# efirdc/Segmentation-Pipeline

Measured on AMD Instinct MI355X. Metric: 3D patches/sec (128³, 4ch) train+infer at 1/2/4/8 MI355X; Dice vs CPU ref, higher is better.
Workload: dtype f32 (tensors, results and accumulation; the products of the 3x3x3 convolutions with >= 8 input channels run as six bf16 MFMAs on an EXACT three-way bf16 split of both f32 operands -- error vs f64 equal to the f32 MFMA kernels', profiles/r04_f32x3_accuracy.txt; the same step on v_mfma_f32_32x32x2_f32

## Files before the change

### include/m355seg.h

```cpp
#ifndef M355SEG_H
#define M355SEG_H

#include <stddef.h>
#include <stdint.h>

#ifdef __cplusplus
extern "C" {
#endif

#define M355_ABI_VERSION 3

enum {
  M355_OK = 0,
  M355_EINVALID_ARG = -1,
  M355_EUNSUPPORTED = -2,
  M355_ELAUNCH = -3,
  M355_EWORKSPACE = -4
};

enum { M355_F32 = 0 };

enum { M355_COMPUTE_F32 = 0, M355_COMPUTE_BF16 = 1, M355_COMPUTE_F16 = 2, M355_COMPUTE_F32X3 = 3 };

enum { M355_ACT_NONE = 0, M355_ACT_RELU = 1, M355_ACT_LEAKY_RELU = 2, M355_ACT_ELU = 3, M355_ACT_GELU = 4,
// ... 65 lines not shown
                               size_t workspace_bytes, void* stream);

int m355_conv3d_plan(const m355_conv3d_desc* d, int32_t which, int32_t* out4);

int m355_conv3d_launch_plan(int32_t entry, const m355_conv3d_desc* d, const int64_t* batch_strides, const uint64_t* pointers,
                            size_t workspace_bytes, int64_t* out12);

size_t m355_conv3d_bwd_data_workspace(const m355_conv3d_desc* d);
int m355_conv3d_bwd_data(const m355_conv3d_desc* d, const float* dy, const float* w,
                         float* dx, void* workspace, size_t workspace_bytes, void* stream);

size_t m355_conv3d_bwd_weight_workspace(const m355_conv3d_desc* d);
int m355_conv3d_bwd_weight(const m355_conv3d_desc* d, const float* x, const float* dy,
                           float* dw, float* dbias,
                           void* workspace, size_t workspace_bytes, void* stream);

size_t m355_conv_transpose3d_workspace(const m355_conv3d_desc* d);
int m355_conv_transpose3d_fwd(const m355_conv3d_desc* d, const float* x, const float* w,
                              const float* bias, float* y,
                              void* workspace, size_t workspace_bytes, void* stream);
int m355_conv_transpose3d_bwd_data(const m355_conv3d_desc* d, const float* dy, const float* w,
                                   float* dx, void* workspace, size_t workspace_bytes,
                                   void* stream);
int m355_conv_transpose3d_bwd_weight(const m355_conv3d_desc* d, const float* x, const float* dy,
                                     float* dw, float* dbias,
                                     void* workspace, size_t workspace_bytes, void* stream);

int m355_conv_transpose3d_plan(const m355_conv3d_desc* d, int32_t which, const void* y_side, int32_t* out4);

int32_t m355_conv_transpose3d_x3_bwd_supported(const m355_conv3d_desc* d, const void* y_side);
// ... 521 lines not shown
```

### segmentation-pipeline_amd/_lib.py

```python
import ctypes as C
import os

_HERE = os.path.dirname(os.path.abspath(__file__))
LIB_PATH = os.environ.get("M355_LIB_PATH") or os.path.join(_HERE, "libm355seg.so")

M355_OK = 0
M355_EUNSUPPORTED = -2
ACT_NONE, ACT_RELU, ACT_LEAKY_RELU = 0, 1, 2
ACT_ELU, ACT_GELU, ACT_GELU_TANH, ACT_SILU = 3, 4, 5, 6
COMPUTE_F32, COMPUTE_BF16, COMPUTE_F16, COMPUTE_F32X3 = 0, 1, 2, 3
CONV_W_PACKED, CONV_SOFTMAX, CONV_SIGMOID = 1, 2, 4


class ConvDesc(C.Structure):
    _fields_ = [
        ("N", C.c_int32), ("Cin", C.c_int32), ("Cout", C.c_int32),
        ("D", C.c_int32), ("H", C.c_int32), ("W", C.c_int32),
        ("k", C.c_int32), ("stride", C.c_int32), ("pad", C.c_int32), ("out_pad", C.c_int32),
        ("x_batch_stride", C.c_int64), ("y_batch_stride", C.c_int64),
        ("compute", C.c_int32), ("flags", C.c_int32),
    ]


class PackItem(C.Structure):
# ... 163 lines not shown
    "m355_upsample_trilinear2x_fwd_h16": (C.c_int, [_P, _P, _i32, _i32, _i32, _i32, _i32, _i64, _i64, _i32, _P]),
    "m355_upsample_trilinear2x_bwd_h16": (C.c_int, [_P, _P, _i32, _i32, _i32, _i32, _i32, _i64, _i64, _i32, _P]),
    "m355_act16_channel_scale": (C.c_int, [_P, _P, _P, _i32, _i32, _i64, _i64, _i64, _i32, _P]),
    "m355_space_to_depth2_h16": (C.c_int, [_P, _P, _i32, _i32, _i32, _i32, _i32, _i64, _i64, _i32, _P]),
    "m355_depth_to_space2_h16": (C.c_int, [_P, _P, _i32, _i32, _i32, _i32, _i32, _i64, _i64, _i32, _P]),
    "m355_conv_transpose3d_h16_bwd_supported": (_i32, [_CD]),
    "m355_conv_transpose3d_h16_bwd_workspace": (_sz, [_CD]),
    "m355_conv_transpose3d_bwd_data_h16": (C.c_int, [_CD, _P, _i64, _P, _P, _i64, _i32, _P]),
    "m355_conv_transpose3d_bwd_weight_h16": (C.c_int, [_CD, _P, _i64, _P, _i64, _P, _P, _f32, _i32, _P, _sz, _P]),
    "m355_conv3d_plan": (C.c_int, [_CD, _i32, C.POINTER(C.c_int32)]),
    "m355_conv3d_launch_plan": (C.c_int, [_i32, _CD, C.POINTER(_i64), C.POINTER(C.c_uint64), _sz, C.POINTER(_i64)]),
    "m355_conv3d_bwd_data_workspace": (_sz, [_CD]),
    "m355_conv3d_bwd_data": (C.c_int, [_CD, _P, _P, _P, _P, _sz, _P]),
    "m355_conv3d_bwd_weight_workspace": (_sz, [_CD]),
    "m355_conv3d_bwd_weight": (C.c_int, [_CD, _P, _P, _P, _P, _P, _sz, _P]),
    "m355_conv_transpose3d_workspace": (_sz, [_CD]),
    "m355_conv_transpose3d_plan": (C.c_int, [_CD, _i32, _P, C.POINTER(C.c_int32)]),
    "m355_conv_transpose3d_fwd": (C.c_int, [_CD, _P, _P, _P, _P, _P, _sz, _P]),
    "m355_conv_transpose3d_bwd_data": (C.c_int, [_CD, _P, _P, _P, _P, _sz, _P]),
    "m355_conv_transpose3d_bwd_weight": (C.c_int, [_CD, _P, _P, _P, _P, _P, _sz, _P]),
    "m355_conv_transpose3d_fwd_h16": (C.c_int, [_CD, _P, _i64, _P, _P, _P, _i64, _i32, _P]),
    "m355_conv_transpose3d_x3_bwd_supported": (_i32, [_CD, _P]),
    "m355_conv_transpose3d_x3_bwd_workspace": (_sz, [_CD]),
    "m355_conv_transpose3d_x3_bwd_plan": (C.c_int, [_CD, _i32, _P, C.POINTER(C.c_int32)]),
    "m355_conv_transpose3d_bwd_data_x3": (C.c_int, [_CD, _P, _P, _P, _P, _sz, _P]),
    "m355_conv_transpose3d_bwd_weight_x3": (C.c_int, [_CD, _P, _P, _P, _P, _P, _sz, _P]),
    "m355_norm_num_stats": (_i64, [_ND]),
    "m355_norm_workspace": (_sz, [_ND]),
    "m355_norm_plan": (C.c_int, [_ND, _i32, C.POINTER(C.c_int32)]),
    "m355_norm_stats": (C.c_int, [_ND, _P, _P, _P, _P, _P, _f32, _P, _sz, _P]),
# ... 226 lines not shown
```

### segmentation-pipeline_amd/csrc/abi.cpp

```cpp
#include "common.hpp"
#include <map>
#include <mutex>
#include <tuple>
#include <utility>

namespace m355 {
static thread_local char g_err[512] = "";
void set_error(const char* fmt, ...) {
  va_list ap;
  va_start(ap, fmt);
  vsnprintf(g_err, sizeof(g_err), fmt, ap);
  va_end(ap);
}

static int env_int(const char* name, int dflt) {
  const char* v = getenv(name);
  if (!v || !*v) return dflt;
  return atoi(v);
}
static Tuning read_tuning() {
  Tuning t;
  t.conv_ntw = env_int("M355_CONV_NTW", 0);
  t.conv_ksplit = env_int("M355_CONV_KSPLIT", 0);
  t.conv_slots = env_int("M355_CONV_SLOTS", 0);
  t.conv_persistent = env_int("M355_CONV_PERSISTENT", 1);
  t.no_small = env_int("M355_NO_SMALL", 0);
  t.smallcout_valu = env_int("M355_SMALLCOUT_VALU", 1);
  t.f32x3 = env_int("M355_F32X3", 1);
  t.f32x3_bww = env_int("M355_F32X3_BWW", 1);
  t.f32x3_edge = env_int("M355_F32X3_EDGE", 0);
  t.f32x3_convt = env_int("M355_F32X3_CONVT", 1);
  t.f32x3_convt_bwd = env_int("M355_F32X3_CONVT_BWD", 1);
  t.bww_nsplit = env_int("M355_BWW_NSPLIT", 0);
  t.bww_gen = env_int("M355_BWW_GEN", 2);
  t.bww_queue = env_int("M355_BWW_QUEUE", 1);
  t.h16_persistent = env_int("M355_H16_PERSISTENT", 1);
  t.tile16 = env_int("M355_TILE16", 1);
  t.convt_h16 = env_int("M355_CONVT_H16", 1);
  t.h16_w8 = env_int("M355_H16_W8", 1);
  t.h16_oneshot = env_int("M355_H16_ONESHOT", 1);
  t.h16_xcd = env_int("M355_H16_XCD", 1);
  t.conv_cube = env_int("M355_CONV_CUBE", 3);
  t.h16_order = env_int("M355_H16_ORDER", 3);
  t.fuse_softmax = env_int("M355_FUSE_SOFTMAX", 1);
  t.convt_wgs = env_int("M355_CONVT_WGS", 0);
  t.h16_stagger = env_int("M355_H16_STAGGER", 2);
  return t;
// ... 104 lines not shown
```

### segmentation-pipeline_amd/csrc/common.hpp

```cpp
#pragma once
#include <hip/hip_runtime.h>
#include <stdint.h>
#include <stdio.h>
#include <stdarg.h>
#include <stdlib.h>
#include <algorithm>
#include "../../include/m355seg.h"

namespace m355 {

void set_error(const char* fmt, ...);

static inline int64_t ceil_div(int64_t a, int64_t b) { return (a + b - 1) / b; }
static inline int64_t round_up(int64_t a, int64_t b) { return ceil_div(a, b) * b; }

static inline int check_launch(const char* what) {
  hipError_t e = hipGetLastError();
  if (e != hipSuccess) {
    set_error("%s: launch failed: %s", what, hipGetErrorString(e));
    return M355_ELAUNCH;
  }
  return M355_OK;
}

// ... 31 lines not shown
  }
  return r;
}

__device__ __forceinline__ float sigmoid_f32(float v) { return 1.f / (1.f + expf(-v)); }

struct Tuning {
  int conv_ntw = 0, conv_ksplit = 0, conv_slots = 0, conv_persistent = 1;
  int no_small = 0, smallcout_valu = 1, bww_nsplit = 0, bww_gen = 2, bww_queue = 1, h16_persistent = 1, tile16 = 1, convt_h16 = 1, h16_w8 = 1, h16_oneshot = 1, h16_xcd = 1;
  int conv_cube = 3, h16_order = 3;
  int fuse_softmax = 1;
  int f32x3 = 1;
  int f32x3_bww = 1;
  int f32x3_edge = 0;
  int f32x3_convt = 1;
  int f32x3_convt_bwd = 1;
  int convt_wgs = 0;
  int h16_stagger = 2;
};
const Tuning& tuning();

static inline int64_t dense_or(int64_t stride, int64_t dense) { return stride ? stride : dense; }

int num_cus();

int* queue_state(hipStream_t st);
int* overflow_flag();

}
```

### segmentation-pipeline_amd/csrc/conv3d.hip

```cpp
#include "conv3d_common.hpp"

namespace m355 {

__global__ void pack_w3_kernel(const float* __restrict__ w, float* __restrict__ wp, int Cout,
                               int Cin, int kin_pad, int mout_pad, int transpose, int* __restrict__ counter) {
  if (counter && blockIdx.x == 0 && threadIdx.x < 16) counter[threadIdx.x] = 0;
  pack_w3_body(w, wp, Cout, Cin, kin_pad, mout_pad, transpose, blockIdx.x, gridDim.x);
}

template <int NTW, int GX>
__global__ __launch_bounds__(256, 1) void conv3_mfma_fwd_kernel(
    const float* __restrict__ x, const float* __restrict__ wp, const float* __restrict__ bias,
    const float* __restrict__ add, float* __restrict__ y, float* __restrict__ slab, int Cin,
    int Cout, int D, int H, int W, int cout_pad, int ty_tiles, int tx_tiles, int nchunks,
    int ksplit, int64_t xbs, int64_t ybs, int64_t slab_stride, float* __restrict__ stat, int otiles, int order) {
  using T = FwdTile<NTW, GX>;
  constexpr int GY = T::GY, TZ = T::TZ, TY = T::TY, TX = T::TX, RS = T::RS, PS = T::PS,
                CS = T::CS, CC = T::CC;
  constexpr int XE = CC * CS;
  constexpr int XPER = (XE + 255) / 256;
  constexpr int WE4 = CC * 27 * 8;
  constexpr int WPER = (WE4 + 255) / 256;
  __shared__ float xs[2][XE];
  __shared__ __attribute__((aligned(16))) float ws[2][CC * 27 * 32];
// ... 1500 lines not shown
    } else {
      for (int64_t s = begin + threadIdx.x; s < end; s += 256) part += p[s];
    }
    acc += part;
  }
  const double tot = block_sum<double, 256>(acc, scratch);
  if (threadIdx.x == 0) partial[(int64_t)o * nblk + b] = tot;
}
__global__ void dbias_finalize_kernel(const double* __restrict__ partial, float* __restrict__ dbias,
                                      int Cout, int nblk) {
  const int o = blockIdx.x * blockDim.x + threadIdx.x;
  if (o >= Cout) return;
  double acc = 0.0;
  for (int b = 0; b < nblk; ++b) acc += partial[(int64_t)o * nblk + b];
  dbias[o] = (float)acc;
}

__global__ void conv3d_direct_fwd_kernel(const float* __restrict__ x, const float* __restrict__ w,
                                         const float* __restrict__ bias,
                                         const float* __restrict__ add, float* __restrict__ y,
                                         int N, int Cin, int Cout, int D, int H, int W, int OD,
                                         int OH, int OW, int k, int stride, int pad, int64_t xbs,
                                         int64_t ybs) {
  const int64_t OS = (int64_t)OD * OH * OW;
  const int64_t total = (int64_t)N * Cout * OS;
  const int k3 = k * k * k;
  for (int64_t i = blockIdx.x * (int64_t)blockDim.x + threadIdx.x; i < total;
       i += (int64_t)gridDim.x * blockDim.x) {
    const int ox = (int)(i % OW);
    int64_t r = i / OW;
// ... 274 lines not shown
    if (int rc = launch_pack_act16((const float*)dy, dy16, d->N, d->Cout, S, r.dy_bs, r.ybs, d->compute, st)) return rc;
    x = x16;
    dy = dy16;
  }
  switch (r.kind) {
    case BwwKind::Direct:
      hipLaunchKernelGGL(conv3d_direct_bwd_weight_kernel, r.grid, dim3(256), 0, st, (const float*)x, (const float*)dy, c.dw,
                         d->N, d->Cin, d->Cout, d->D, d->H, d->W, out_dim(d->D, d->k, d->stride, d->pad),
                         out_dim(d->H, d->k, d->stride, d->pad), out_dim(d->W, d->k, d->stride, d->pad), d->k, d->stride,
                         d->pad, r.xbs, r.ybs);
      break;
    case BwwKind::X3:
    case BwwKind::X3c:
      launch_bww_x3(r, (const float*)x, (const float*)dy, slab, d, st);
      break;
    case BwwKind::C8:
    case BwwKind::C8Small:
      launch_bww_c8(r, x, dy, slab, d, st);
      if (int rc = check_launch(r.kind == BwwKind::C8 ? "conv3_bww_c8" : "conv3_bww_c8_small")) return rc;
      break;
    default:
      if (r.plan.gx == 32) launch_bww_mfma<32>(r, (const float*)x, (const float*)dy, slab, d, st);
      else if (r.plan.gx == 16) launch_bww_mfma<16>(r, (const float*)x, (const float*)dy, slab, d, st);
      else launch_bww_mfma<8>(r, (const float*)x, (const float*)dy, slab, d, st);
  }
  if (r.aux & (AUX_SLAB_T | AUX_SLAB_TAP))
    launch_slab_reduce_t(r, slab, c.dw, d->Cin, d->Cout, c.grad_unscale, st);
  else if (r.aux & AUX_SLAB_PLAIN)
    hipLaunchKernelGGL(slab_reduce_kernel, r.reduce_grid, dim3(r.reduce_block), 0, st, slab, c.dw, (int64_t)d->Cout * d->Cin * 27,
                       r.plan.nsplit);
  void* dbias_ws = (char*)c.ws + r.dbias_off;
  if (r.aux & AUX_DBIAS_C8) {
    if (int rc = launch_dbias_c8(dy, r.ybs, c.dbias, d->N, d->Cout, S, d->compute, c.grad_unscale, dbias_ws, st)) return rc;
  } else if (r.aux & AUX_DBIAS_F32) {
    launch_dbias(c.dy32, c.dbias, d->N, d->Cout, out_voxels(d), r.dy_bs, dbias_ws, st);
  }
  return check_launch(r.who);
}

}

int launch_dbias(const float* dy, float* dbias, int N, int Cout, int64_t S, int64_t ybs, void* ws, hipStream_t st) {
  const int nblk = (int)m355::ceil_div(S, m355::DBIAS_CHUNK);
  if (S % 4 == 0 && ybs % 4 == 0 && ((uintptr_t)dy & 15) == 0)
    hipLaunchKernelGGL(m355::dbias_partial_kernel<true>, dim3((unsigned)nblk, (unsigned)Cout), dim3(256), 0, st, dy,
                       (double*)ws, N, S, ybs, nblk);
  else
    hipLaunchKernelGGL(m355::dbias_partial_kernel<false>, dim3((unsigned)nblk, (unsigned)Cout), dim3(256), 0, st, dy,
                       (double*)ws, N, S, ybs, nblk);
  hipLaunchKernelGGL(m355::dbias_finalize_kernel, dim3((unsigned)m355::ceil_div(Cout, 64)), dim3(64), 0, st,
                     (const double*)ws, dbias, Cout, nblk);
  return M355_OK;
}
```

### segmentation-pipeline_amd/csrc/conv3d_common.hpp

```cpp
#pragma once
#include "common.hpp"
#include "h16.hpp"
#include "conv3d_route.hpp"

namespace m355 {


__device__ __forceinline__ int opaque(int v) {
  asm volatile("" : "+v"(v));
  return v;
}

__device__ __forceinline__ void queue_leave(int* __restrict__ counter) {
  if (threadIdx.x == 0) {
    if (atomicAdd(counter + 8, 1) == (int)gridDim.x - 1) {
#pragma unroll
      for (int r = 0; r < 9; ++r) counter[r] = 0;
    }
  }
}

template <int NTW, int GX>
struct FwdTile {
  static constexpr int GY = 32 / GX;
// ... 202 lines not shown
                   float* slab, const m355_conv3d_desc* d, hipStream_t st, float* stat);

struct BwwCall {
  const m355_conv3d_desc* d;
  const void* x;
  const void* dy;
  const float* dy32;
  float* dw;
  float* dbias;
  float grad_unscale;
  void* ws;
  hipStream_t st;
};
int launch_bww(const BwwRoute& r, const BwwCall& c);
void launch_bww_x3(const BwwRoute& r, const float* x, const float* dy, float* slab, const m355_conv3d_desc* d, hipStream_t st);
void launch_bww_c8(const BwwRoute& r, const void* x16, const void* dy16, float* slab, const m355_conv3d_desc* d, hipStream_t st);

struct PackEntry {
  const float* w;
  void* wp;
  int* counter;
  int Cout, Cin;
  int kdim;
  int mout_pad;
  int transpose, kind;
  int blk0, nblk;
};
constexpr int PACK_BATCH = 64;
struct PackBatch {
  PackEntry e[PACK_BATCH];
// ... 25 lines not shown
    if (!transpose) {
      if (kc < Cin && m < Cout) v = w[((int64_t)m * Cin + kc) * 27 + tap];
    } else {
      if (kc < Cout && m < Cin) v = w[((int64_t)kc * Cin + m) * 27 + (26 - tap)];
    }
    wp[i] = v;
  }
}
__global__ void splitk_reduce_kernel(const float* __restrict__ slab, const float* __restrict__ bias,
                                     const float* __restrict__ add, float* __restrict__ y, int N,
                                     int Cout, int64_t S, int ksplit, int64_t slab_stride,
                                     int64_t ybs);

}

int launch_dbias(const float* dy, float* dbias, int N, int Cout, int64_t S, int64_t ybs, void* ws, hipStream_t st);
```

### segmentation-pipeline_amd/csrc/conv3d_f32x3.hip

```cpp
#include "conv3d_common.hpp"

namespace m355 {

typedef __bf16 bf16x8 __attribute__((ext_vector_type(8)));
typedef unsigned u32x4 __attribute__((ext_vector_type(4)));

constexpr int X3_PAIRS = 14;
constexpr int X3_QUADS = 7;
__host__ __device__ constexpr int x3_pair_tap(int pair, int half) {
  return pair < 9 ? pair * 3 + half : (pair < 12 ? (pair - 9) * 9 + half * 3 + 2 : (pair == 12 ? half * 9 + 8 : 26));
}

__device__ __forceinline__ void x3_split(float v, unsigned& hi, unsigned& mid, unsigned& lo) {
  const unsigned u = __float_as_uint(v);
  hi = u & 0xffff0000u;
  const float r1 = (u & 0x7f800000u) == 0x7f800000u ? 0.f : v - __uint_as_float(hi);
  mid = __float_as_uint(r1) & 0xffff0000u;
  lo = __float_as_uint(r1 - __uint_as_float(mid));
}
__device__ __forceinline__ unsigned x3_pack(unsigned a, unsigned b) { return __builtin_amdgcn_perm(b, a, 0x07060302u); }

__device__ __forceinline__ void pack_w3_x3_item(const float* __restrict__ w, u32x4* __restrict__ wq, int64_t i, int Cout_w,
                                                int Cin_w, int kin, int mout, int nchunks, int transpose) {
  const int lane = (int)(i & 63);
// ... 924 lines not shown
static void launch_bww_x3_t(const BwwRoute& r, const float* x, const float* dy, float* slab, const m355_conv3d_desc* d,
                            hipStream_t st) {
  const BwwX3Plan& p = r.x3;
  if (r.kind == BwwKind::X3c)
    hipLaunchKernelGGL((conv3_bww_x3c_kernel<TX>), r.grid, dim3(512), 0, st, x, dy, slab, d->N, d->Cin, d->Cout, d->D, d->H,
                       d->W, p.ty_tiles, p.tx_tiles, p.k, r.xbs, r.ybs);
  else
    hipLaunchKernelGGL((conv3_bww_x3_kernel<TX>), r.grid, dim3(512), 0, st, x, dy, slab, d->N, d->Cin, d->Cout, d->D, d->H,
                       d->W, p.ty_tiles, p.tx_tiles, p.nsplit, p.ctiles, p.otiles, r.xbs, r.ybs);
}

void launch_bww_x3(const BwwRoute& r, const float* x, const float* dy, float* slab, const m355_conv3d_desc* d, hipStream_t st) {
  if (r.x3.tx == 32) launch_bww_x3_t<32>(r, x, dy, slab, d, st);
  else if (r.x3.tx == 16) launch_bww_x3_t<16>(r, x, dy, slab, d, st);
  else launch_bww_x3_t<8>(r, x, dy, slab, d, st);
}

template <int NVT>
__global__ __launch_bounds__(256) void convt_k2s2_fwd_x3_kernel(
    const float* __restrict__ x, const float* __restrict__ w, const float* __restrict__ bias, float* __restrict__ y, int Cin,
    int Cout, int D, int H, int W, int64_t xbs, int64_t ybs, int mt_per_wg) {
  extern __shared__ __attribute__((aligned(16))) unsigned char xs3_raw[];
  u32x4* xs3 = reinterpret_cast<u32x4*>(xs3_raw);
  constexpr int NG = NVT / 32, P = 256 / NVT;
  const int tid = threadIdx.x, lane = tid & 63;
  const int wave = __builtin_amdgcn_readfirstlane(tid >> 6);
  const int half = lane >> 5, l32 = lane & 31;
  const int S = D * H * W;
  const int v0 = blockIdx.x * NVT;
  const int n = blockIdx.z;
// ... 303 lines not shown
```

### segmentation-pipeline_amd/csrc/conv3d_host.hip

```cpp
#include "conv3d_common.hpp"

using namespace m355;

static ConvRoute query_conv(const m355_conv3d_desc* d, int which) { return route_conv(d, conv_query_args(which)); }
static BwwRoute query_bww(const m355_conv3d_desc* d) { return route_bww(d, conv_query_args(2)); }
static BwwRoute query_bww_c8(const m355_conv3d_desc* d) {
  ConvArgs a{};
  a.entry = CE_BWD_WEIGHT_H16;
  return route_bww_c8(d, a);
}

extern "C" size_t m355_conv3d_fwd_workspace(const m355_conv3d_desc* d) { return d ? query_conv(d, 0).workspace_bytes : 0; }
extern "C" size_t m355_conv3d_bwd_data_workspace(const m355_conv3d_desc* d) { return d ? query_conv(d, 1).workspace_bytes : 0; }
extern "C" size_t m355_conv3d_h16_workspace(const m355_conv3d_desc* d, int32_t which) {
  return d ? query_conv(d, which).h16_workspace_bytes : 0;
}
extern "C" size_t m355_conv3d_bwd_weight_workspace(const m355_conv3d_desc* d) { return d ? query_bww(d).workspace_bytes : 0; }
extern "C" size_t m355_conv3d_bwd_weight_h16_workspace(const m355_conv3d_desc* d) {
  return d ? query_bww_c8(d).h16_workspace_bytes : 0;
}
extern "C" size_t m355_conv3d_bwd_weight_c8_workspace(const m355_conv3d_desc* d) {
  return d ? query_bww_c8(d).c8_workspace_bytes : 0;
}
extern "C" size_t m355_conv3d_packed_bytes(const m355_conv3d_desc* d, int32_t which) {
// ... 175 lines not shown
  return run_bww({CE_BWD_WEIGHT, P(x), P(dy), 0, 0, P(dw), P(dbias), P(workspace), workspace_bytes, {0, 0}}, d, 1.f, stream);
}

extern "C" int m355_conv3d_bwd_weight_h16(const m355_conv3d_desc* d, const void* x16, int64_t x16_batch_stride,
                                          const void* dy16, int64_t dy16_batch_stride, const float* dy, float* dw,
                                          float* dbias, void* workspace, size_t workspace_bytes, void* stream) {
  return run_bww({CE_BWD_WEIGHT_H16, P(x16), P(dy16), P(dy), 0, P(dw), P(dbias), P(workspace), workspace_bytes,
                  {x16_batch_stride, dy16_batch_stride}}, d, 1.f, stream);
}

extern "C" int m355_conv3d_bwd_weight_c8(const m355_conv3d_desc* d, const void* x16, int64_t x16_batch_stride,
                                         const void* dy16, int64_t dy16_batch_stride, float* dw, float* dbias,
                                         float grad_unscale, void* workspace, size_t workspace_bytes, void* stream) {
  return run_bww({CE_BWD_WEIGHT_C8, P(x16), P(dy16), 0, 0, P(dw), P(dbias), P(workspace), workspace_bytes,
                  {x16_batch_stride, dy16_batch_stride}}, d, grad_unscale, stream);
}

extern "C" int m355_conv3d_launch_plan(int32_t entry, const m355_conv3d_desc* d, const int64_t* batch_strides,
                                       const uint64_t* pointers, size_t workspace_bytes, int64_t* out12) {
  M355_REQUIRE(entry >= 0 && entry < CE_COUNT && batch_strides && pointers && out12, M355_EINVALID_ARG,
               "conv3d_launch_plan: bad entry point index / null pointer");
  const ConvArgs a = {entry, (uintptr_t)pointers[0], (uintptr_t)pointers[1], (uintptr_t)pointers[2], (uintptr_t)pointers[3],
                      (uintptr_t)pointers[4], (uintptr_t)pointers[5], (uintptr_t)pointers[6], workspace_bytes,
                      {batch_strides[0], batch_strides[1]}};
  if (entry == CE_BWD_WEIGHT || entry == CE_BWD_WEIGHT_H16 || entry == CE_BWD_WEIGHT_C8) {
    BwwRoute r;
    if (int rc = check_bww(a, d, &r)) return rc;
    const int64_t o[12] = {(int64_t)r.kind, r.grid.x, r.grid.y, r.grid.z, r.block, 0, 0, r.aux, (int64_t)r.need, r.reduce_grid.x,
                           (int64_t)r.dbias_off, (int64_t)r.x16_off};
    std::copy_n(o, 12, out12);
// ... 10 lines not shown
```

### segmentation-pipeline_amd/csrc/conv3d_route.hpp

```cpp
#pragma once
#include "h16.hpp"

namespace m355 {

inline bool is16(int compute) { return compute == M355_COMPUTE_BF16 || compute == M355_COMPUTE_F16; }
inline int out_dim(int in, int k, int s, int p) { return (in + 2 * p - k) / s + 1; }
inline int64_t splitk_c8_slots(int64_t S) { return std::max<int64_t>(1, std::min<int64_t>(ceil_div(S, 256), 2048)); }
constexpr int SMALLCOUT_TZ_K = 90, SMALLCOUT_VS_TZ = 4, SMALLCOUT_VS_TY = 8, SMALLCOUT_VS_TX = 64;
inline size_t smallcout_packed_bytes(int Cin) { return (size_t)round_up((int64_t)round_up(Cin, 2) * SMALLCOUT_TZ_K * 32 * 4, 256); }

struct FwdPlan {
  bool mfma;
  bool persistent;
  int gx, ntw;
  int tz_tiles, ty_tiles, tx_tiles;
  int otiles, kin_pad, mout_pad, nchunks, ksplit;
  int tile16;
  int nw;
  int oneshot;
  int x3;
  int64_t slots;
  size_t wp_bytes, slab_bytes;
};
struct BwwClasses {
// ... 388 lines not shown
  a.entry = which == 0 ? CE_FWD : (which == 2 ? CE_BWD_WEIGHT : CE_BWD_DATA);
  return a;
}

enum ConvAux : uint32_t {
  AUX_PACK_W = 1,
  AUX_PACK_IN = 2,
  AUX_PACK_DY = 4,
  AUX_TILE16 = 8,
  AUX_SPLITK = 16,
  AUX_SPLITK_STATS = 32,
  AUX_SLAB_T = 64,
  AUX_SLAB_TAP = 128,
  AUX_SLAB_PLAIN = 256,
  AUX_DBIAS_F32 = 512,
  AUX_DBIAS_C8 = 1024
};

enum class ConvKind {
  Direct,
  MfmaF32,
  MfmaF32Queue,
  SmallCoutValu,
  SmallCoutToeplitz,
  X3,
  H16Queue, H16Queue8, H16OneShot,
  H16C4,
  H16Cout4
};
inline bool is_h16(ConvKind k) { return k >= ConvKind::H16Queue; }
inline bool is_smallcout(ConvKind k) { return k == ConvKind::SmallCoutValu || k == ConvKind::SmallCoutToeplitz; }
// ... 201 lines not shown
  M355_REQUIRE(!r.sigmoid || (r.mout <= 4 && r.plan.ksplit == 1 && !a.add && !a.stat && !r.out16), M355_EUNSUPPORTED,
               "conv3d(16-bit operands): the sigmoid epilogue needs Cout <= 4, an unsplit plan, fp32 output, no add / statistics");
  return M355_OK;
}

enum class BwwKind {
  Direct,
  MfmaVec,
  MfmaScalar,
  Mfma2,
  Mfma2c,
  Small,
  X3,
  X3c,
  C8,
  C8Small
};
struct BwwRoute {
  BwwKind kind;
  bool via_pack;
  bool h16, ok;
  BwwPlan plan;
  BwwX3Plan x3;
  int nsplit;
  dim3 grid;
  int block;
  BwwClasses kred;
  int reduce_ctiles;
  dim3 reduce_grid;
  int reduce_block;
  uint32_t aux;
// ... 128 lines not shown
    for (int c = 0; c < 4; ++c) r.kred.ns[c] = p.nsplit;
  } else {
    r.kind = vec ? BwwKind::MfmaVec : BwwKind::MfmaScalar;
    r.grid = dim3((unsigned)p.ctiles, (unsigned)p.otiles, (unsigned)p.nsplit);
  }
  if (gen2) {
    route_slab_reduce_t(r, d->Cout, p.ctiles);
  } else {
    r.aux |= AUX_SLAB_PLAIN;
    r.reduce_grid = dim3((unsigned)std::min<int64_t>(ceil_div(total, 64), 4096));
    r.reduce_block = 64;
  }
  return r;
}

static inline int check_bww(const ConvArgs& a, const m355_conv3d_desc* d, BwwRoute* route) {
  const char* who = CONV_ENTRY_NAMES[a.entry];
  if (int rc = validate_conv(d, who)) return rc;
  const int64_t S = (int64_t)d->D * d->H * d->W;
  if (a.entry == CE_BWD_WEIGHT) {
    M355_REQUIRE(a.in && a.w && a.out, M355_EINVALID_ARG, "conv3d_bwd_weight: null pointer");
    const BwwRoute& r = *route = route_bww(d, a);
    M355_REQUIRE(a.ws && a.ws_bytes >= r.need, M355_EWORKSPACE, "conv3d_bwd_weight: workspace too small (%zu < %zu)",
                 a.ws_bytes, r.need);
    M355_REQUIRE(r.kind == BwwKind::Direct || r.kind == BwwKind::X3 || r.kind == BwwKind::X3c ||
                     ((int64_t)d->Cin * S < (1ll << 31) && (int64_t)d->Cout * S < (1ll << 31)),
                 M355_EUNSUPPORTED, "conv3d_bwd_weight: tensor exceeds 2^31 elements per sample");
    if (r.via_pack)
      M355_REQUIRE((a.ws & 15) == 0, M355_EINVALID_ARG, "conv3d_bwd_weight_h16: c8 tensor not 16B aligned");
    else if (r.kind == BwwKind::Direct)
// ... 21 lines not shown
```

### segmentation-pipeline_amd/ops.py

```python
import ctypes as C
import os
import weakref
from dataclasses import dataclass
from typing import List, NamedTuple, Optional, Sequence

import numpy as np
import torch

from . import _lib
from ._lib import ACT_LEAKY_RELU, ACT_NONE, ACT_RELU, ConvDesc, NormDesc, check

FP32_SPLIT = os.environ.get("M355_FP32_SPLIT", "1") != "0"
_COMPUTE = {"fp32": _lib.COMPUTE_F32X3 if FP32_SPLIT else _lib.COMPUTE_F32, "fp32_mfma": _lib.COMPUTE_F32,
            "bf16": _lib.COMPUTE_BF16, "fp16": _lib.COMPUTE_F16}
_DT16 = {_lib.COMPUTE_BF16: torch.bfloat16, _lib.COMPUTE_F16: torch.float16}
_compute_mode = "fp32"


def set_precision(mode: str):
    global _compute_mode
    if mode not in _COMPUTE:
        raise ValueError(f"precision must be one of {sorted(_COMPUTE)}, not {mode!r}")
    _compute_mode = mode

# ... 11 lines not shown
    def __init__(self, mode):
        self.mode = mode

    def __enter__(self):
        self.prev = get_precision()
        set_precision(self.mode)

    def __exit__(self, *exc):
        set_precision(self.prev)


CONV_PROFILE: Optional[list] = None
CONV_PROFILE_KEYS: Optional[set] = None
CONV_PROFILE_EVERY = 1
_prof_seen = 0


def _conv_bytes(N, Cin, Cout, voxels, taps, in_elem, out_elem):
    return float(N) * voxels * (Cin * in_elem + Cout * out_elem) + 4.0 * Cin * Cout * taps


def _conv_launch(tag, d, which, in_elem, out_elem, fn, *args):
    prof = CONV_PROFILE
    if prof is not None:
        plan = conv_plan(d, which) if which is not None else None
        if CONV_PROFILE_KEYS is not None and (tag, plan) not in CONV_PROFILE_KEYS:
            prof = None
        elif CONV_PROFILE_EVERY > 1:
            global _prof_seen
            _prof_seen += 1
# ... 1010 lines not shown
            x16 = Act16(x, *ctx.x16)
            x_dtype, x_device = ctx.x_meta
            dy16 = _c8_twin(dy, x16.compute)
            if dy16 is None:
                dy16 = pack_act16(dy, x16.compute)
        else:
            x_dtype, x_device = x.dtype, x.device
        if need_w or (need_b and ctx.has_bias):
            dw = torch.empty_like(weight)
            db = torch.empty(d.Cout, dtype=weight.dtype, device=weight.device) if ctx.has_bias else None
            if x16 is not None:
                ws = _workspace(L.m355_conv3d_bwd_weight_h16_workspace(C.byref(d)), x_device)
                _conv_launch("conv3d_bwd_weight", d, None, 4, 4, L.m355_conv3d_bwd_weight_h16, C.byref(d), x16.ptr(),
                             x16.batch_stride(), dy16.ptr(), dy16.batch_stride(), _p(dy) if db is not None else None,
                             _p(dw), _p(db), _p(ws), ws.numel(), _stream())
            else:
                ws = _workspace(L.m355_conv3d_bwd_weight_workspace(C.byref(d)), x_device)
                _conv_launch("conv3d_bwd_weight", d, 2, 4, 4, L.m355_conv3d_bwd_weight, C.byref(d), _p(x), _p(dy),
                             _p(dw), _p(db), _p(ws), ws.numel(), _stream())
        if need_x:
            dx = torch.empty((d.N, d.Cin, d.D, d.H, d.W), dtype=x_dtype, device=x_device)
            dd = _conv_desc(d.N, d.Cin, d.Cout, d.D, d.H, d.W, d.k, d.stride, d.pad, 0, d.y_batch_stride, compute=d.compute)
            wbuf, flags = _packed_weight(weight, dd, 1)
            ddk = _with_flags(dd, flags)
            if dy16 is not None:
                ws = _workspace(L.m355_conv3d_h16_workspace(C.byref(dd), 1), x_device)
                _conv_launch("conv3d_bwd_data", dd, 1, 4, 4, L.m355_conv3d_bwd_data_h16, C.byref(ddk), dy16.ptr(),
                             dy16.batch_stride(), _p(wbuf), _p(dx), _p(ws), ws.numel(), _stream())
            else:
                ws = _workspace(L.m355_conv3d_bwd_data_workspace(C.byref(dd)), x_device)
                _conv_launch("conv3d_bwd_data", dd, 1, 4, 4, L.m355_conv3d_bwd_data, C.byref(ddk), _p(dy), _p(wbuf),
# ... 1871 lines not shown
```

Baseline: 52.09.

## Add split-bf16 MFMA weight-gradient kernel for few-channel edge 3x3x3 convolutions

Adds a new backward-weight kernel for 3x3x3 stride-1 convolutions where one side has at most 4 channels, such as the input and output edge layers. It splits both f32 operands into three bf16 parts and accumulates six bf16 MFMAs per product, staging tiles in LDS with transposed reads and prefetching the next tile while computing. It is routed in by default for F32X3 compute above a voxel floor, replacing the generic fp32 path that is likely inefficient for tiny channel counts. It also adds a block-parallel dbias finalize kernel; the trade-offs are extra per-split slab workspace and a reduction pass.

New measurement: 52.55 (median of 6 runs). Within noise of the previous version (+0.9%).

```diff
diff --git a/include/m355seg.h b/include/m355seg.h
--- a/include/m355seg.h
+++ b/include/m355seg.h
@@ -103,6 +103,12 @@
 int m355_conv3d_bwd_weight(const m355_conv3d_desc* d, const float* x, const float* dy,
                            float* dw, float* dbias,
                            void* workspace, size_t workspace_bytes, void* stream);
+
+int32_t m355_conv3d_edge_x3_bwd_supported(const m355_conv3d_desc* d, const void* x, const void* dy);
+size_t m355_conv3d_edge_x3_bwd_workspace(const m355_conv3d_desc* d);
+int m355_conv3d_edge_x3_bwd_plan(const m355_conv3d_desc* d, const void* x, const void* dy, int32_t* out4);
+int m355_conv3d_bwd_weight_edge_x3(const m355_conv3d_desc* d, const float* x, const float* dy, float* dw, float* dbias,
+                                   void* workspace, size_t workspace_bytes, void* stream);
 
 size_t m355_conv_transpose3d_workspace(const m355_conv3d_desc* d);
 int m355_conv_transpose3d_fwd(const m355_conv3d_desc* d, const float* x, const float* w,
diff --git a/segmentation-pipeline_amd/_lib.py b/segmentation-pipeline_amd/_lib.py
--- a/segmentation-pipeline_amd/_lib.py
+++ b/segmentation-pipeline_amd/_lib.py
@@ -201,6 +201,10 @@
     "m355_conv3d_bwd_data": (C.c_int, [_CD, _P, _P, _P, _P, _sz, _P]),
     "m355_conv3d_bwd_weight_workspace": (_sz, [_CD]),
     "m355_conv3d_bwd_weight": (C.c_int, [_CD, _P, _P, _P, _P, _P, _sz, _P]),
+    "m355_conv3d_edge_x3_bwd_supported": (_i32, [_CD, _P, _P]),
+    "m355_conv3d_edge_x3_bwd_workspace": (_sz, [_CD]),
+    "m355_conv3d_edge_x3_bwd_plan": (C.c_int, [_CD, _P, _P, C.POINTER(C.c_int32)]),
+    "m355_conv3d_bwd_weight_edge_x3": (C.c_int, [_CD, _P, _P, _P, _P, _P, _sz, _P]),
     "m355_conv_transpose3d_workspace": (_sz, [_CD]),
     "m355_conv_transpose3d_plan": (C.c_int, [_CD, _i32, _P, C.POINTER(C.c_int32)]),
     "m355_conv_transpose3d_fwd": (C.c_int, [_CD, _P, _P, _P, _P, _P, _sz, _P]),
diff --git a/segmentation-pipeline_amd/csrc/abi.cpp b/segmentation-pipeline_amd/csrc/abi.cpp
--- a/segmentation-pipeline_amd/csrc/abi.cpp
+++ b/segmentation-pipeline_amd/csrc/abi.cpp
@@ -31,6 +31,7 @@
   t.f32x3_edge = env_int("M355_F32X3_EDGE", 0);
   t.f32x3_convt = env_int("M355_F32X3_CONVT", 1);
   t.f32x3_convt_bwd = env_int("M355_F32X3_CONVT_BWD", 1);
+  t.f32x3_edge_bww = env_int("M355_F32X3_EDGE_BWW", 1);
   t.bww_nsplit = env_int("M355_BWW_NSPLIT", 0);
   t.bww_gen = env_int("M355_BWW_GEN", 2);
   t.bww_queue = env_int("M355_BWW_QUEUE", 1);
diff --git a/segmentation-pipeline_amd/csrc/common.hpp b/segmentation-pipeline_amd/csrc/common.hpp
--- a/segmentation-pipeline_amd/csrc/common.hpp
+++ b/segmentation-pipeline_amd/csrc/common.hpp
@@ -69,6 +69,7 @@
   int f32x3_bww = 1;
   int f32x3_edge = 0;
   int f32x3_convt = 1;
+  int f32x3_edge_bww = 1;
   int f32x3_convt_bwd = 1;
   int convt_wgs = 0;
   int h16_stagger = 2;
diff --git a/segmentation-pipeline_amd/csrc/conv3d.hip b/segmentation-pipeline_amd/csrc/conv3d.hip
--- a/segmentation-pipeline_amd/csrc/conv3d.hip
+++ b/segmentation-pipeline_amd/csrc/conv3d.hip
@@ -1538,6 +1538,22 @@
   double acc = 0.0;
   for (int b = 0; b < nblk; ++b) acc += partial[(int64_t)o * nblk + b];
   dbias[o] = (float)acc;
+}
+
+__global__ __launch_bounds__(256) void dbias_finalize_par_kernel(const double* __restrict__ partial, float* __restrict__ dbias,
+                                                                 int nblk) {
+  __shared__ double red[256];
+  const int o = blockIdx.x, t = threadIdx.x;
+  double acc = 0.0;
+  for (int b = t; b < nblk; b += 256) acc += partial[(int64_t)o * nblk + b];
+  red[t] = acc;
+  __syncthreads();
+#pragma unroll
+  for (int w = 128; w >= 1; w >>= 1) {
+    if (t < w) red[t] += red[t + w];
+    __syncthreads();
+  }
+  if (t == 0) dbias[o] = (float)red[0];
 }
 
 __global__ void conv3d_direct_fwd_kernel(const float* __restrict__ x, const float* __restrict__ w,
@@ -1842,6 +1858,9 @@
     case BwwKind::X3c:
       launch_bww_x3(r, (const float*)x, (const float*)dy, slab, d, st);
       break;
+    case BwwKind::X3Small:
+      launch_bww_x3_small(r, (const float*)x, (const float*)dy, slab, d, st);
+      break;
     case BwwKind::C8:
     case BwwKind::C8Small:
       launch_bww_c8(r, x, dy, slab, d, st);
@@ -1861,14 +1880,14 @@
   if (r.aux & AUX_DBIAS_C8) {
     if (int rc = launch_dbias_c8(dy, r.ybs, c.dbias, d->N, d->Cout, S, d->compute, c.grad_unscale, dbias_ws, st)) return rc;
   } else if (r.aux & AUX_DBIAS_F32) {
-    launch_dbias(c.dy32, c.dbias, d->N, d->Cout, out_voxels(d), r.dy_bs, dbias_ws, st);
+    launch_dbias(c.dy32, c.dbias, d->N, d->Cout, out_voxels(d), r.dy_bs, dbias_ws, st, (r.aux & AUX_DBIAS_PAR) != 0);
   }
   return check_launch(r.who);
 }
 
 }
 
-int launch_dbias(const float* dy, float* dbias, int N, int Cout, int64_t S, int64_t ybs, void* ws, hipStream_t st) {
+int launch_dbias(const float* dy, float* dbias, int N, int Cout, int64_t S, int64_t ybs, void* ws, hipStream_t st, bool par) {
   const int nblk = (int)m355::ceil_div(S, m355::DBIAS_CHUNK);
   if (S % 4 == 0 && ybs % 4 == 0 && ((uintptr_t)dy & 15) == 0)
     hipLaunchKernelGGL(m355::dbias_partial_kernel<true>, dim3((unsigned)nblk, (unsigned)Cout), dim3(256), 0, st, dy,
@@ -1876,7 +1895,10 @@
   else
     hipLaunchKernelGGL(m355::dbias_partial_kernel<false>, dim3((unsigned)nblk, (unsigned)Cout), dim3(256), 0, st, dy,
                        (double*)ws, N, S, ybs, nblk);
-  hipLaunchKernelGGL(m355::dbias_finalize_kernel, dim3((unsigned)m355::ceil_div(Cout, 64)), dim3(64), 0, st,
-                     (const double*)ws, dbias, Cout, nblk);
+  if (par)
+    hipLaunchKernelGGL(m355::dbias_finalize_par_kernel, dim3((unsigned)Cout), dim3(256), 0, st, (const double*)ws, dbias, nblk);
+  else
+    hipLaunchKernelGGL(m355::dbias_finalize_kernel, dim3((unsigned)m355::ceil_div(Cout, 64)), dim3(64), 0, st,
+                       (const double*)ws, dbias, Cout, nblk);
   return M355_OK;
 }
diff --git a/segmentation-pipeline_amd/csrc/conv3d_common.hpp b/segmentation-pipeline_amd/csrc/conv3d_common.hpp
--- a/segmentation-pipeline_amd/csrc/conv3d_common.hpp
+++ b/segmentation-pipeline_amd/csrc/conv3d_common.hpp
@@ -240,6 +240,8 @@
 };
 int launch_bww(const BwwRoute& r, const BwwCall& c);
 void launch_bww_x3(const BwwRoute& r, const float* x, const float* dy, float* slab, const m355_conv3d_desc* d, hipStream_t st);
+void launch_bww_x3_small(const BwwRoute& r, const float* x, const float* dy, float* slab, const m355_conv3d_desc* d,
+                         hipStream_t st);
 void launch_bww_c8(const BwwRoute& r, const void* x16, const void* dy16, float* slab, const m355_conv3d_desc* d, hipStream_t st);
 
 struct PackEntry {
@@ -295,4 +297,5 @@
 
 }
 
-int launch_dbias(const float* dy, float* dbias, int N, int Cout, int64_t S, int64_t ybs, void* ws, hipStream_t st);
+int launch_dbias(const float* dy, float* dbias, int N, int Cout, int64_t S, int64_t ybs, void* ws, hipStream_t st,
+                 bool par = false);
diff --git a/segmentation-pipeline_amd/csrc/conv3d_f32x3.hip b/segmentation-pipeline_amd/csrc/conv3d_f32x3.hip
--- a/segmentation-pipeline_amd/csrc/conv3d_f32x3.hip
+++ b/segmentation-pipeline_amd/csrc/conv3d_f32x3.hip
@@ -962,6 +962,208 @@
   if (r.x3.tx == 32) launch_bww_x3_t<32>(r, x, dy, slab, d, st);
   else if (r.x3.tx == 16) launch_bww_x3_t<16>(r, x, dy, slab, d, st);
   else launch_bww_x3_t<8>(r, x, dy, slab, d, st);
+}
+
+__device__ __forceinline__ bf16x8 x3_tr_frag_q(const unsigned char* p) {
+  typedef __attribute__((address_space(3))) x3_s16x4 lds_s16x4;
+  const x3_s16x4 lo = __builtin_amdgcn_ds_read_tr16_b64_v4i16((lds_s16x4*)(p));
+  const x3_s16x4 hi = __builtin_amdgcn_ds_read_tr16_b64_v4i16((lds_s16x4*)(p + 32));
+  return __builtin_bit_cast(bf16x8, __builtin_shufflevector(lo, hi, 0, 1, 2, 3, 4, 5, 6, 7));
+}
+
+__global__ __launch_bounds__(256, 2) void conv3_bww_x3_small_kernel(
+    const float* __restrict__ P, const float* __restrict__ Q, float* __restrict__ slab, int N, int CP, int CQ, int D, int H,
+    int W, int tz_tiles, int ty_tiles, int tx_tiles, int nsplit, int ptiles, int64_t pbs, int64_t qbs, int swap, int Cin,
+    int Cout) {
+  constexpr int TZ = 2, TY = 4, TX = 32, NV = TZ * TY * TX;
+  constexpr int HR = TX + 2, HP = (TY + 2) * HR, HVX = (TZ + 2) * HP;
+  constexpr int QPER = (HVX + 255) / 256;
+  constexpr int QR = 40, QP = (TY + 2) * QR + 8;
+  constexpr int PPLANE = NV * 64, QPLANE = (TZ + 2) * QP * 8;
+  unsigned OOB = 0x80000000u;
+  asm volatile("" : "+s"(OOB));
+  __shared__ __attribute__((aligned(16))) unsigned char smem[3 * PPLANE + 3 * QPLANE];
+  unsigned char* const ps = smem;
+  unsigned char* const qs = smem + 3 * PPLANE;
+  const int tid = threadIdx.x, lane = tid & 63;
+  const int wave = __builtin_amdgcn_readfirstlane(tid >> 6);
+  const int half = lane >> 5, l32 = lane & 31;
+  int vid;
+  {
+    const int nwg = (int)gridDim.x, bid = (int)blockIdx.x;
+    const int q = nwg >> 3, r = nwg & 7, xcd = bid & 7;
+    vid = (xcd < r ? xcd * (q + 1) : r * (q + 1) + (xcd - r) * q) + (bid >> 3);
+  }
+  const int ptile = vid % ptiles, split = vid / ptiles;
+  const int iHW = H * W, S = D * iHW;
+  const int nch = min(32, CP - 32 * ptile);
+  int qrel[QPER], qlds[QPER];
+  unsigned qcode[QPER];
+#pragma unroll
+  for (int k = 0; k < QPER; ++k) {
+    const int hv = tid + 256 * k;
+    const int zz = hv / HP, r = hv - zz * HP;
+    const int yy = r / HR, xx = r - yy * HR;
+    qrel[k] = zz * iHW + yy * W + xx;
+    qlds[k] = (zz * QP + yy * QR + xx) * 8;
+    qcode[k] = hv < HVX ? (1u << zz) | (1u << (8 + yy)) | ((unsigned)xx << 16) : 0xffffu;
+  }
+  const int dvz = tid / (TY * TX), dvy = (tid / TX) % TY, dvx = tid % TX;
+  const int tiles_per_n = tz_tiles * ty_tiles * tx_tiles;
+  const int ntiles = N * tiles_per_n;
+  __amdgpu_buffer_rsrc_t rp, rq;
+  unsigned zymask = 0u;
+  int qbase = 0, pbase = 0, xlim = 0;
+  bool pok = false;
+  auto tile_setup = [&](int tile, bool live) __attribute__((always_inline)) {
+    int t = tile;
+    const int n = t / tiles_per_n;
+    t -= n * tiles_per_n;
+    const int txt = t % tx_tiles;
+    t /= tx_tiles;
+    const int tyt = t % ty_tiles, tzt = t / ty_tiles;
+    const int z0 = tzt * TZ, y0 = tyt * TY, x0 = txt * TX;
+    rp = __builtin_amdgcn_make_buffer_rsrc((void*)(P + (int64_t)n * pbs + (int64_t)(32 * ptile) * S), 0, live ? nch * S * 4 : 0,
+                                           0x00020000);
+    rq = __builtin_amdgcn_make_buffer_rsrc((void*)(Q + (int64_t)n * qbs), 0, live ? CQ * S * 4 : 0, 0x00020000);
+    zymask = 0u;
+    for (int zz = 0; zz < TZ + 2; ++zz)
+      if (z0 + zz - 1 >= 0 && z0 + zz - 1 < D) zymask |= 1u << zz;
+    for (int yy = 0; yy < TY + 2; ++yy)
+      if (y0 + yy - 1 >= 0 && y0 + yy - 1 < H) zymask |= 1u << (8 + yy);
+    qbase = (z0 - 1) * iHW + (y0 - 1) * W + x0 - 1;
+    xlim = x0 - 1;
+    const int gz = z0 + dvz, gy = y0 + dvy, gx = x0 + dvx;
+    pok = gz < D && gy < H && gx < W;
+    pbase = gz * iHW + gy * W + gx;
+  };
+  float pr[32], qr[QPER][4];
+  auto fetch = [&]() __attribute__((always_inline)) {
+#pragma unroll
+    for (int k = 0; k < QPER; ++k) {
+      const int xx = (int)(qcode[k] >> 16);
+      const bool ok = ((qcode[k] & 0xffffu) & ~zymask) == 0u && (unsigned)(xlim + xx) < (unsigned)W;
+#pragma unroll
+      for (int q = 0; q < 4; ++q)
+        qr[k][q] = __builtin_bit_cast(float, __builtin_amdgcn_raw_buffer_load_b32(
+                                                 rq, ok ? (unsigned)(q * S + qbase + qrel[k]) * 4u : OOB, 0, 0));
+    }
+#pragma unroll
+    for (int c = 0; c < 32; ++c)
+      pr[c] = __builtin_bit_cast(float, __builtin_amdgcn_raw_buffer_load_b32(rp, pok ? (unsigned)(c * S + pbase) * 4u : OOB, 0, 0));
+  };
+  auto commit = [&]() __attribute__((always_inline)) {
+#pragma unroll
+    for (int k = 0; k < QPER; ++k) {
+      const int hv = tid + 256 * k;
+      unsigned h[4], m[4], l[4];
+#pragma unroll
+      for (int q = 0; q < 4; ++q) x3_split(qr[k][q], h[q], m[q], l[q]);
+      if (hv < HVX) {
+        *reinterpret_cast<uint2*>(qs + qlds[k]) = make_uint2(x3_pack(h[0], h[1]), x3_pack(h[2], h[3]));
+        *reinterpret_cast<uint2*>(qs + QPLANE + qlds[k]) = make_uint2(x3_pack(m[0], m[1]), x3_pack(m[2], m[3]));
+        *reinterpret_cast<uint2*>(qs + 2 * QPLANE + qlds[k]) = make_uint2(x3_pack(l[0], l[1]), x3_pack(l[2], l[3]));
+      }
+    }
+#pragma unroll
+    for (int g = 0; g < 4; ++g) {
+      unsigned h[8], m[8], l[8];
+#pragma unroll
+      for (int j = 0; j < 8; ++j) x3_split(pr[8 * g + j], h[j], m[j], l[j]);
+      unsigned char* row = ps + tid * 64 + g * 16;
+      *reinterpret_cast<uint4*>(row) = make_uint4(x3_pack(h[0], h[1]), x3_pack(h[2], h[3]), x3_pack(h[4], h[5]), x3_pack(h[6], h[7]));
+      *reinterpret_cast<uint4*>(row + PPLANE) = make_uint4(x3_pack(m[0], m[1]), x3_pack(m[2], m[3]), x3_pack(m[4], m[5]), x3_pack(m[6], m[7]));
+      *reinterpret_cast<uint4*>(row + 2 * PPLANE) = make_uint4(x3_pack(l[0], l[1]), x3_pack(l[2], l[3]), x3_pack(l[4], l[5]), x3_pack(l[6], l[7]));
+    }
+  };
+  const int grp = lane >> 4, tq = (lane & 15) >> 2, tp = lane & 3;
+  const unsigned char* pb = ps + (8 * (grp >> 1) + tq) * 64 + (grp & 1) * 32 + tp * 8;
+  int qoff[4];
+#pragma unroll
+  for (int g = 0; g < 4; ++g) {
+    const int tau = min(g * 8 + 4 * (grp & 1) + tp, 26);
+    const int tsrc = swap ? 26 - tau : tau;
+    qoff[g] = ((tsrc / 9) * QP + ((tsrc / 3) % 3) * QR + tsrc % 3 + 8 * (grp >> 1) + tq) * 8;
+  }
+  f32x16 acc[4];
+#pragma unroll
+  for (int g = 0; g < 4; ++g)
+#pragma unroll
+    for (int r = 0; r < 16; ++r) acc[g][r] = 0.f;
+  if (split < ntiles) {
+    tile_setup(split, true);
+    fetch();
+    commit();
+  }
+  __syncthreads();
+  for (int tile = split; tile < ntiles; tile += nsplit) {
+    const bool more = tile + nsplit < ntiles;
+    tile_setup(more ? tile + nsplit : tile, more);
+    fetch();
+    __builtin_amdgcn_sched_barrier(0);
+#pragma unroll
+    for (int ks = 0; ks < 4; ++ks) {
+      const int row = wave * 2 + (ks >> 1), xk = ks & 1;
+      const unsigned char* a0 = pb + (row * TX + 16 * xk) * 64;
+      const unsigned char* q0 = qs + ((row >> 2) * QP + (row & 3) * QR + 16 * xk) * 8;
+      const bf16x8 ah = x3_tr_frag(a0), am = x3_tr_frag(a0 + PPLANE), al = x3_tr_frag(a0 + 2 * PPLANE);
+      bf16x8 bh[4], bm[4], bl[4];
+#pragma unroll
+      for (int g = 0; g < 4; ++g) {
+        bh[g] = x3_tr_frag_q(q0 + qoff[g]);
+        bm[g] = x3_tr_frag_q(q0 + qoff[g] + QPLANE);
+        bl[g] = x3_tr_frag_q(q0 + qoff[g] + 2 * QPLANE);
+      }
+#pragma unroll
+      for (int g = 0; g < 4; ++g) acc[g] = __builtin_amdgcn_mfma_f32_32x32x16_bf16(al, bh[g], acc[g], 0, 0, 0);
+#pragma unroll
+      for (int g = 0; g < 4; ++g) acc[g] = __builtin_amdgcn_mfma_f32_32x32x16_bf16(am, bh[g], acc[g], 0, 0, 0);
+#pragma unroll
+      for (int g = 0; g < 4; ++g) acc[g] = __builtin_amdgcn_mfma_f32_32x32x16_bf16(ah, bh[g], acc[g], 0, 0, 0);
+#pragma unroll
+      for (int g = 0; g < 4; ++g) acc[g] = __builtin_amdgcn_mfma_f32_32x32x16_bf16(am, bm[g], acc[g], 0, 0, 0);
+#pragma unroll
+      for (int g = 0; g < 4; ++g) acc[g] = __builtin_amdgcn_mfma_f32_32x32x16_bf16(ah, bm[g], acc[g], 0, 0, 0);
+#pragma unroll
+      for (int g = 0; g < 4; ++g) acc[g] = __builtin_amdgcn_mfma_f32_32x32x16_bf16(ah, bl[g], acc[g], 0, 0, 0);
+    }
+    __syncthreads();
+    if (more) commit();
+    __syncthreads();
+  }
+  float* red = reinterpret_cast<float*>(smem);
+#pragma unroll
+  for (int g = 0; g < 4; ++g)
+#pragma unroll
+    for (int r = 0; r < 16; ++r) red[((g * 4 + wave) * 16 + r) * 64 + lane] = acc[g][r];
+  __syncthreads();
+  float sum[16];
+#pragma unroll
+  for (int r = 0; r < 16; ++r) {
+    const float* p = red + ((wave * 4) * 16 + r) * 64 + lane;
+    sum[r] = ((p[0] + p[16 * 64]) + p[2 * 16 * 64]) + p[3 * 16 * 64];
+  }
+  float* sl = slab + (int64_t)split * 27 * Cout * Cin;
+  const int tap = wave * 8 + (l32 >> 2), q = l32 & 3;
+  if (tap < 27 && q < CQ) {
+#pragma unroll
+    for (int r = 0; r < 16; ++r) {
+      const int pch = ptile * 32 + (r & 3) + 8 * (r >> 2) + 4 * half;
+      if (pch < CP) {
+        const int o = swap ? q : pch, c = swap ? pch : q;
+        sl[((int64_t)tap * Cout + o) * Cin + c] = sum[r];
+      }
+    }
+  }
+}
+
+void launch_bww_x3_small(const BwwRoute& r, const float* x, const float* dy, float* slab, const m355_conv3d_desc* d,
+                         hipStream_t st) {
+  const int swap = d->Cin <= 4 ? 0 : 1;
+  const int CP = swap ? d->Cin : d->Cout, CQ = swap ? d->Cout : d->Cin;
+  hipLaunchKernelGGL(conv3_bww_x3_small_kernel, r.grid, dim3(256), 0, st, swap ? x : dy, swap ? dy : x, slab, d->N, CP, CQ, d->D,
+                     d->H, d->W, (int)ceil_div(d->D, 2), (int)ceil_div(d->H, 4), (int)ceil_div(d->W, 32), r.nsplit,
+                     (int)ceil_div(CP, 32), swap ? r.xbs : r.ybs, swap ? r.ybs : r.xbs, swap, d->Cin, d->Cout);
 }
 
 template <int NVT>
diff --git a/segmentation-pipeline_amd/csrc/conv3d_host.hip b/segmentation-pipeline_amd/csrc/conv3d_host.hip
--- a/segmentation-pipeline_amd/csrc/conv3d_host.hip
+++ b/segmentation-pipeline_amd/csrc/conv3d_host.hip
@@ -213,6 +213,47 @@
                                          float grad_unscale, void* workspace, size_t workspace_bytes, void* stream) {
   return run_bww({CE_BWD_WEIGHT_C8, P(x16), P(dy16), 0, 0, P(dw), P(dbias), P(workspace), workspace_bytes,
                   {x16_batch_stride, dy16_batch_stride}}, d, grad_unscale, stream);
+}
+
+static BwwRoute query_bww_edge_x3(const m355_conv3d_desc* d, const void* x, const void* dy) {
+  ConvArgs a{};
+  a.entry = CE_BWD_WEIGHT;
+  a.in = P(x);
+  a.w = P(dy);
+  return route_bww_edge_x3(d, a);
+}
+static bool edge_x3_desc_ok(const m355_conv3d_desc* d) {
+  return d && d->N > 0 && d->Cin > 0 && d->Cout > 0 && d->D > 0 && d->H > 0 && d->W > 0;
+}
+extern "C" int32_t m355_conv3d_edge_x3_bwd_supported(const m355_conv3d_desc* d, const void* x, const void* dy) {
+  return edge_x3_desc_ok(d) && query_bww_edge_x3(d, x, dy).ok ? 1 : 0;
+}
+extern "C" size_t m355_conv3d_edge_x3_bwd_workspace(const m355_conv3d_desc* d) {
+  return edge_x3_desc_ok(d) ? query_bww_edge_x3(d, nullptr, nullptr).workspace_bytes : 0;
+}
+extern "C" int m355_conv3d_edge_x3_bwd_plan(const m355_conv3d_desc* d, const void* x, const void* dy, int32_t* out4) {
+  if (int rc = validate_conv(d, "conv3d_edge_x3_bwd_plan")) return rc;
+  M355_REQUIRE(out4, M355_EINVALID_ARG, "conv3d_edge_x3_bwd_plan: null pointer");
+  std::copy_n(query_bww_edge_x3(d, x, dy).plan_code, 4, out4);
+  return M355_OK;
+}
+extern "C" int m355_conv3d_bwd_weight_edge_x3(const m355_conv3d_desc* d, const float* x, const float* dy, float* dw, float* dbias,
+                                              void* workspace, size_t workspace_bytes, void* stream) {
+  const char* who = "conv3d_bwd_weight_edge_x3";
+  if (int rc = validate_conv(d, who)) return rc;
+  M355_REQUIRE(x && dy && dw, M355_EINVALID_ARG, "%s: null pointer", who);
+  const ConvArgs a = {CE_BWD_WEIGHT, P(x), P(dy), 0, 0, P(dw), P(dbias), P(workspace), workspace_bytes, {0, 0}};
+  const BwwRoute r = route_bww_edge_x3(d, a);
+  M355_REQUIRE(r.ok, M355_EUNSUPPORTED,
+               "%s: needs M355_COMPUTE_F32X3, kernel_size 3 / stride 1 / padding 1, at most 4 channels on one side, below 2^24 "
+               "voxels and 2^29 elements per sample, 4-byte aligned operands, a batch above the router's floor, and M355_F32X3 / "
+               "M355_F32X3_EDGE_BWW != 0 (m355_conv3d_edge_x3_bwd_supported): take m355_conv3d_bwd_weight", who);
+  const size_t need = dbias ? r.workspace_bytes : r.slab_bytes;
+  M355_REQUIRE(workspace && workspace_bytes >= need, M355_EWORKSPACE, "%s: workspace too small (%zu < %zu)", who,
+               workspace_bytes, need);
+  M355_REQUIRE((P(workspace) & 7) == 0, M355_EINVALID_ARG, "%s: workspace not 8-byte aligned", who);
+  const BwwCall c = {d, x, dy, dy, dw, dbias, 1.f, workspace, (hipStream_t)stream};
+  return launch_bww(r, c);
 }
 
 extern "C" int m355_conv3d_launch_plan(int32_t entry, const m355_conv3d_desc* d, const int64_t* batch_strides,
diff --git a/segmentation-pipeline_amd/csrc/conv3d_route.hpp b/segmentation-pipeline_amd/csrc/conv3d_route.hpp
--- a/segmentation-pipeline_amd/csrc/conv3d_route.hpp
+++ b/segmentation-pipeline_amd/csrc/conv3d_route.hpp
@@ -426,7 +426,8 @@
   AUX_SLAB_TAP = 128,
   AUX_SLAB_PLAIN = 256,
   AUX_DBIAS_F32 = 512,
-  AUX_DBIAS_C8 = 1024
+  AUX_DBIAS_C8 = 1024,
+  AUX_DBIAS_PAR = 2048
 };
 
 enum class ConvKind {
@@ -658,7 +659,8 @@
   X3,
   X3c,
   C8,
-  C8Small
+  C8Small,
+  X3Small
 };
 struct BwwRoute {
   BwwKind kind;
@@ -817,6 +819,42 @@
   return r;
 }
 
+constexpr int64_t EDGE_X3_BWW_MIN_VOXELS = 65536;
+static inline BwwRoute route_bww_edge_x3(const m355_conv3d_desc* d, const ConvArgs& a) {
+  BwwRoute r{};
+  r.who = "conv3d_bwd_weight_edge_x3";
+  r.kind = BwwKind::Direct;
+  r.block = 256;
+  r.grid = r.reduce_grid = dim3(0, 0, 0);
+  const int64_t S = (int64_t)d->D * d->H * d->W;
+  if (d->compute != M355_COMPUTE_F32X3 || !tuning().f32x3 || !tuning().f32x3_edge_bww) return r;
+  if (!is_k3s1p1(d) || (d->Cin > 4 && d->Cout > 4)) return r;
+  if ((int64_t)std::max(d->Cin, d->Cout) * S >= (1ll << 29) || S >= (1ll << 24)) return r;
+  if (((a.in | a.w) & 3) != 0) return r;
+  if ((int64_t)d->N * S < EDGE_X3_BWW_MIN_VOXELS && tuning().f32x3_edge_bww < 2) return r;
+  const int64_t ntiles = (int64_t)d->N * ceil_div(d->D, 2) * ceil_div(d->H, 4) * ceil_div(d->W, 32);
+  if (ntiles >= (1ll << 31)) return r;
+  r.ok = true;
+  r.kind = BwwKind::X3Small;
+  const int ptiles = (int)ceil_div(d->Cin <= 4 ? d->Cout : d->Cin, 32);
+  int64_t nsplit = std::max<int64_t>(1, 2 * (int64_t)num_cus() / ptiles);
+  if (const int force = tuning().bww_nsplit) nsplit = force;
+  r.nsplit = (int)std::min<int64_t>(nsplit, ntiles);
+  r.grid = dim3((unsigned)(ptiles * r.nsplit));
+  r.xbs = dense_or(d->x_batch_stride, (int64_t)d->Cin * S);
+  r.ybs = r.dy_bs = dense_or(d->y_batch_stride, (int64_t)d->Cout * S);
+  const int ctiles = (int)ceil_div(d->Cin, 32), otiles = (int)ceil_div(d->Cout, 32);
+  r.kred.of = otiles;
+  r.kred.cf = ctiles;
+  for (int c = 0; c < 4; ++c) r.kred.ns[c] = r.nsplit;
+  route_slab_reduce_t(r, d->Cout, ctiles);
+  if (a.stat) r.aux |= AUX_DBIAS_F32 | AUX_DBIAS_PAR;
+  r.slab_bytes = r.dbias_off = (size_t)round_up((int64_t)r.nsplit * d->Cout * d->Cin * 27 * 4, 256);
+  r.workspace_bytes = r.need = r.slab_bytes + dbias_ws_bytes(d->Cout, S);
+  r.plan_code[0] = 12; r.plan_code[1] = ptiles; r.plan_code[2] = r.nsplit; r.plan_code[3] = 0;
+  return r;
+}
+
 static inline int check_bww(const ConvArgs& a, const m355_conv3d_desc* d, BwwRoute* route) {
   const char* who = CONV_ENTRY_NAMES[a.entry];
   if (int rc = validate_conv(d, who)) return rc;
diff --git a/segmentation-pipeline_amd/ops.py b/segmentation-pipeline_amd/ops.py
--- a/segmentation-pipeline_amd/ops.py
+++ b/segmentation-pipeline_amd/ops.py
@@ -49,6 +49,7 @@
 CONV_PROFILE_KEYS: Optional[set] = None
 CONV_PROFILE_EVERY = 1
 _prof_seen = 0
+edge_x3_counts = {"edge_x3": 0, "plain": 0}
 
 
 def _conv_bytes(N, Cin, Cout, voxels, taps, in_elem, out_elem):
@@ -1089,7 +1090,13 @@
                 _conv_launch("conv3d_bwd_weight", d, None, 4, 4, L.m355_conv3d_bwd_weight_h16, C.byref(d), x16.ptr(),
                              x16.batch_stride(), dy16.ptr(), dy16.batch_stride(), _p(dy) if db is not None else None,
                              _p(dw), _p(db), _p(ws), ws.numel(), _stream())
+            elif d.compute == _lib.COMPUTE_F32X3 and L.m355_conv3d_edge_x3_bwd_supported(C.byref(d), _p(x), _p(dy)):
+                edge_x3_counts["edge_x3"] += 1
+                ws = _workspace(L.m355_conv3d_edge_x3_bwd_workspace(C.byref(d)), x_device)
+                _conv_launch("conv3d_bwd_weight", d, 2, 4, 4, L.m355_conv3d_bwd_weight_edge_x3, C.byref(d), _p(x), _p(dy),
+                             _p(dw), _p(db), _p(ws), ws.numel(), _stream())
             else:
+                edge_x3_counts["plain"] += 1
                 ws = _workspace(L.m355_conv3d_bwd_weight_workspace(C.byref(d)), x_device)
                 _conv_launch("conv3d_bwd_weight", d, 2, 4, 4, L.m355_conv3d_bwd_weight, C.byref(d), _p(x), _p(dy),
                              _p(dw), _p(db), _p(ws), ws.numel(), _stream())
```
